# bkpcoding/distributed_ML_pytorch

Measured on AMD Instinct MI355X. Metric: samples/sec (whole node) ResNet-18 ASGD at 1/2/4/8 MI355X; time-to-target-loss, higher is better.
Workload: dtype bf16; 1 GPU; model=resnet18 (CIFAR stem), global_batch=512, per_gpu_batch=512, image=3x32x32, parallelism=asgd-local-ps x1, n_push=10, n_pull=10, staleness=1, push_combine=sum, hip_graph=True, master_dtype=fp32, wire_dtype=fp32

## Files before the change

### distributed_ml_pytorch_amd/csrc/bind/norm_pool.cpp

```cpp
#include "util.h"

namespace dmp::bind {
namespace {

int64_t channels_of(const Tensor& x) { return x.size(1); }

using OptTensors = std::initializer_list<const optional<Tensor>*>;

void check_bn_stats(const Tensor& stats, int64_t C) {
  TORCH_CHECK(stats.scalar_type() == at::kFloat && stats.numel() == 4 * C,
              "bn: stats must be fp32 [4, C]");
}

struct BnFwd {
  int64_t C, M;
  at::TensorOptions fopt;
  Tensor y, stats, mask;
  std::vector<Tensor> result() const { return {y, stats, mask}; }
};

BnFwd bn_fwd_front(const Tensor& x, const optional<Tensor>& res, OptTensors affine, bool relu,
                   bool want_mask) {
  check_nhwc_bf16(x, "x");
  BnFwd f;
  f.C = channels_of(x);
  f.M = x.numel() / f.C;
  TORCH_CHECK(f.C % 8 == 0 && f.C <= 2048, "bn: C must be a multiple of 8 and <= 2048, got ", f.C);
  if (has(res)) {
    check_nhwc_bf16(*res, "res");
    same_shape(*res, x, "res");
  }
  check_vecs(affine, at::kFloat, f.C, "bn affine / running tensors");
  f.fopt = x.options().dtype(at::kFloat);
  f.y = at::empty_like(x);
  f.stats = at::empty({4, f.C}, f.fopt);
  if (want_mask && relu) f.mask = at::empty({f.M, f.C / 8}, x.options().dtype(at::kByte));
  return f;
}

std::vector<Tensor> bn_fwd(Tensor x, optional<Tensor> res, optional<Tensor> gamma,
                           optional<Tensor> beta, optional<Tensor> running_mean,
                           optional<Tensor> running_var, double momentum, double eps,
                           bool training, bool relu, optional<Tensor> slots, bool want_mask) {
  TORCH_CHECK(training || (has(running_mean) && has(running_var)),
// ... 72 lines not shown
  b.mask = relu_mask_ptr(mask, relu, b.M, b.C);
  b.fopt = x.options().dtype(at::kFloat);
  b.dx = at::empty_like(x);
  if (want_dres) b.dres = at::empty_like(x);
  return b;
}

std::vector<Tensor> bn_bwd(Tensor x, Tensor dy, optional<Tensor> y, optional<Tensor> gamma,
                           Tensor stats, optional<Tensor> dgamma, optional<Tensor> dbeta,
                           bool relu, bool want_dres, optional<Tensor> slots,
                           optional<Tensor> mask, bool batch_stats) {
  auto b = bn_bwd_front(x, dy, y, gamma, stats, dgamma, dbeta, relu, want_dres, mask);
  auto part = bn_slots(slots, b.C, b.fopt);
  auto coef = at::empty({3, b.C}, b.fopt);
  dmp::launch_bn_bwd(bf16(x), bf16(dy), b.y, ptr_or_null<float>(gamma), stats.data_ptr<float>(),
                     ptr_or_null<float>(dgamma), ptr_or_null<float>(dbeta), coef.data_ptr<float>(),
                     part.data_ptr<float>(), bf16(b.dx), bf16_or_null(b.dres), b.M, (int)b.C, relu,
                     cur_stream(), b.mask, batch_stats);
  return b.result();
}

std::vector<Tensor> bn_bwd_fold(Tensor x, Tensor dy, optional<Tensor> y, optional<Tensor> gamma,
                                Tensor stats, optional<Tensor> dgamma, optional<Tensor> dbeta,
                                bool relu, bool want_dres, Tensor slots, optional<Tensor> mask,
                                optional<Tensor> zero_buf) {
  auto b = bn_bwd_front(x, dy, y, gamma, stats, dgamma, dbeta, relu, want_dres, mask);
  auto part = bn_slots(slots, b.C, b.fopt);
  float* zb = other_slots(zero_buf, b.C, b.fopt, part);
  dmp::launch_bn_bwd_fold(bf16(x), bf16(dy), b.y, ptr_or_null<float>(gamma),
                          stats.data_ptr<float>(), ptr_or_null<float>(dgamma),
                          ptr_or_null<float>(dbeta), part.data_ptr<float>(), zb, bf16(b.dx),
                          bf16_or_null(b.dres), b.M, (int)b.C, relu, cur_stream(), b.mask);
  return b.result();
}

std::vector<Tensor> bn_relu_maxpool_fwd(Tensor x, Tensor part, bool have_partials,
                                        optional<Tensor> gamma, optional<Tensor> beta,
                                        optional<Tensor> running_mean,
                                        optional<Tensor> running_var, double momentum, double eps,
                                        optional<Tensor> zero_buf, int64_t K, int64_t S,
                                        int64_t P) {
  check_nhwc_bf16(x, "x");
  TORCH_CHECK(x.dim() == 4, "bn_relu_maxpool expects 4-D input");
  TORCH_CHECK(dmp::guard::bf16_bytes_ok(x.size(0), x.size(2), x.size(3), x.size(1)),
              "bn_relu_maxpool: x over 2 GiB (32-bit offsets)");
  const int N = (int)x.size(0), C = (int)x.size(1), H = (int)x.size(2), W = (int)x.size(3);
  TORCH_CHECK(dmp::bn_maxpool_supported(C, (int)K, (int)S, (int)P),
              "bn_relu_maxpool: needs C % 64 == 0, C <= 2048 and a 3x3/s2/p1 window");
  auto fopt = x.options().dtype(at::kFloat);
  part = bn_slots(part, C, fopt);
  float* zb = other_slots(zero_buf, C, fopt, part);
  check_vecs({&gamma, &beta, &running_mean, &running_var}, at::kFloat, C,
             "bn affine / running tensors");
  const int Ho = dmp::maxpool_out(H, (int)K, (int)S, (int)P);
  const int Wo = dmp::maxpool_out(W, (int)K, (int)S, (int)P);
  TORCH_CHECK(Ho > 0 && Wo > 0, "bn_relu_maxpool: window larger than input");
  auto y = at::empty({N, C, Ho, Wo}, x.options().memory_format(kCL));
  auto idx = at::empty({N, C, Ho, Wo}, x.options().dtype(at::kByte).memory_format(kCL));
  auto xm = at::empty({N, C, Ho, Wo}, x.options().memory_format(kCL));
  auto stats = at::empty({4, C}, fopt);
  dmp::launch_bn_relu_maxpool_fold(
      bf16(x), bf16(y), idx.data_ptr<uint8_t>(), bf16(xm), ptr_or_null<float>(gamma),
      ptr_or_null<float>(beta), ptr_or_null<float>(running_mean), ptr_or_null<float>(running_var),
      stats.data_ptr<float>(), part.data_ptr<float>(), zb, N, H, W, C, (float)momentum, (float)eps,
      have_partials, cur_stream());
  return {y, idx, stats, xm};
// ... 174 lines not shown
  if (!aligned(dy)) dy = dy.clone(mf);
  TORCH_CHECK(dy.sizes() == y.sizes() && dy.scalar_type() == at::kBFloat16, "relu_bwd: dy shape");
  Tensor dst = has(out) ? *out : at::empty_like(dy);
  TORCH_CHECK(dst.sizes() == y.sizes() && dst.is_contiguous(mf) &&
                  dst.scalar_type() == at::kBFloat16,
              "relu_bwd: out layout");
  Tensor dx = aligned(dst) ? dst : at::empty_like(dy);
  dmp::launch_relu_bwd(bf16(dy), bf16(y), bf16(dx), y.numel(), cur_stream());
  if (!dx.is_same(dst)) dst.copy_(dx);
  return dst;
}

}

void bind_norm_pool(pybind11::module_& m) {
  m.def("bn_fold_weights", &bn_fold_weights,
        "inference-time BatchNorm fold: (bf16 w * s, fp32 shift, bf16 shift)", py::arg("w"),
        py::arg("gamma"), py::arg("beta"), py::arg("rmean"), py::arg("rvar"),
        py::arg("cbias") = py::none(), py::arg("eps") = 1e-5);
  m.def("bn_fwd_from_partials", &bn_fwd_from_partials, "BN forward from conv-epilogue partials",
        py::arg("x"), py::arg("part"), py::arg("G"), py::arg("res"), py::arg("gamma"),
        py::arg("beta"), py::arg("running_mean"), py::arg("running_var"), py::arg("momentum"),
        py::arg("eps"), py::arg("relu"), py::arg("want_mask") = false);
  m.def("bn_fwd_fold", &bn_fwd_fold, "BN forward, finalize folded into the apply",
        py::arg("x"), py::arg("part"), py::arg("have_partials"), py::arg("res") = py::none(),
        py::arg("gamma") = py::none(), py::arg("beta") = py::none(),
        py::arg("running_mean") = py::none(), py::arg("running_var") = py::none(),
        py::arg("momentum") = 0.1, py::arg("eps") = 1e-5, py::arg("relu") = false,
        py::arg("want_mask") = false, py::arg("zero_buf") = py::none());
  m.def("bn_bwd_fold", &bn_bwd_fold, "BN backward, finalize folded into the apply",
        py::arg("x"), py::arg("dy"), py::arg("y"), py::arg("gamma"), py::arg("stats"),
        py::arg("dgamma"), py::arg("dbeta"), py::arg("relu"), py::arg("want_dres"),
        py::arg("slots"), py::arg("mask") = py::none(), py::arg("zero_buf") = py::none());
  m.def("bn_maxpool_supported",
        [](int64_t C, int64_t K, int64_t S, int64_t P) {
          return dmp::bn_maxpool_supported((int)C, (int)K, (int)S, (int)P);
        },
        "fused BN + ReLU + max pool applies to (C, K, S, P)");
  m.def("bn_relu_maxpool_fwd", &bn_relu_maxpool_fwd,
        "BN + ReLU + max pool forward, finalize folded in -> (y, idx, stats, x at the taps)",
        py::arg("x"),
        py::arg("part"), py::arg("have_partials"), py::arg("gamma"), py::arg("beta"),
        py::arg("running_mean"), py::arg("running_var"), py::arg("momentum"), py::arg("eps"),
        py::arg("zero_buf"), py::arg("K"), py::arg("S"), py::arg("P"));
  m.def("maxpool_bn_bwd", &maxpool_bn_bwd, "backward of bn_relu_maxpool_fwd -> dx", py::arg("x"),
        py::arg("dp"), py::arg("idx"), py::arg("xm"), py::arg("gamma"), py::arg("stats"), py::arg("dgamma"),
        py::arg("dbeta"), py::arg("slots"), py::arg("zero_buf"), py::arg("K"), py::arg("S"),
        py::arg("P"));
  m.def("bn_fwd", &bn_fwd, "NHWC batchnorm(+residual)(+relu) forward", py::arg("x"),
        py::arg("res"), py::arg("gamma"), py::arg("beta"), py::arg("running_mean"),
        py::arg("running_var"), py::arg("momentum"), py::arg("eps"), py::arg("training"),
        py::arg("relu"), py::arg("slots") = py::none(), py::arg("want_mask") = false);
  m.def("bn_bwd", &bn_bwd, "NHWC batchnorm(+residual)(+relu) backward", py::arg("x"),
        py::arg("dy"), py::arg("y"), py::arg("gamma"), py::arg("stats"), py::arg("dgamma"),
        py::arg("dbeta"), py::arg("relu"), py::arg("want_dres"), py::arg("slots") = py::none(),
        py::arg("mask") = py::none(), py::arg("batch_stats") = true);
  m.def("relu_bwd", &relu_bwd, "ReLU backward from the saved output", py::arg("dy"), py::arg("y"),
        py::arg("out") = py::none());
  m.def("gap_fwd", &gap_fwd, "NHWC global average pool forward");
  m.def("gap_linear_fwd", &gap_linear_fwd, "fused NHWC global average pool + Linear forward",
        py::arg("x"), py::arg("w"), py::arg("bias") = py::none());
  m.def("gap_linear_bwd", &gap_linear_bwd, "fused GAP + Linear backward (dx, dW +=, db +=)",
        py::arg("dy"), py::arg("f"), py::arg("w"), py::arg("gw"), py::arg("gb") = py::none(),
        py::arg("H"), py::arg("W"));
  m.def("gap_linear_supported",
        [](int64_t C, int64_t N) { return dmp::gap_linear_supported((int)C, (int)N); },
// ... 12 lines not shown
```

### distributed_ml_pytorch_amd/csrc/bn.hip

```cpp
#include "common.h"

#include <algorithm>
#include <cstdlib>

namespace dmp {

__device__ __forceinline__ void load8(const u16* p, float v[8]) {
  const bf16x8 r = *reinterpret_cast<const bf16x8*>(p);
#pragma unroll
  for (int k = 0; k < 8; ++k) v[k] = bf2f(r.v[k]);
}

__device__ __forceinline__ void store8(u16* p, const float v[8]) {
  bf16x8 r;
#pragma unroll
  for (int k = 0; k < 8; ++k) r.v[k] = f2bf(v[k]);
  *reinterpret_cast<bf16x8*>(p) = r;
}

__device__ __forceinline__ bf16x8 bn_ldv(const u16* p) { return *reinterpret_cast<const bf16x8*>(p); }
__device__ __forceinline__ void bn_stv(u16* p, const bf16x8& r) { *reinterpret_cast<bf16x8*>(p) = r; }

__device__ __forceinline__ void relu_mask_bits(unsigned bits, float g[8]) {
#pragma unroll
  for (int k = 0; k < 8; ++k) g[k] = (bits >> k) & 1u ? g[k] : 0.f;
}
__device__ __forceinline__ void relu_mask_from_x(const float xv[8], const float* __restrict__ stats,
                                                 int C, int c0, float g[8]) {
#pragma unroll
  for (int k = 0; k < 8; ++k) {
    const float y = fmaxf(bn_pre(xv[k], stats[2 * C + c0 + k], stats[3 * C + c0 + k]), 0.f);
    g[k] = bf2f(f2bf(y)) > 0.f ? g[k] : 0.f;
  }
// ... 656 lines not shown
#define DMP_BN_PART(R)                                                                          \
  hipLaunchKernelGGL((bn_partial_kernel<1, R>), dim3(G), dim3(256), lds, s, x, dy, y, mask, stats, \
                     part, M, C)
  if (mode == 0) DMP_BN_PART(0);
  else if (mode == 1) DMP_BN_PART(1);
  else if (mode == 2) DMP_BN_PART(2);
  else DMP_BN_PART(3);
#undef DMP_BN_PART
  const int cs = fold_cs(C);
  const dim3 grid = fold_grid(M, C, cs);
#define DMP_FOLD_B(CS, R, D)                                                                   \
  hipLaunchKernelGGL((bn_bwd_apply_fold_kernel<CS, R, D>), grid, dim3(256), 0, s, x, dy, y, mask, \
                     part, zero_buf, gamma, stats, dgamma, dbeta, dx, dres, M, C)
#define DMP_FOLD_BV(CS)                                                \
  if (dres) {                                                          \
    if (mode == 0) DMP_FOLD_B(CS, 0, true);                            \
    else if (mode == 1) DMP_FOLD_B(CS, 1, true);                       \
    else if (mode == 2) DMP_FOLD_B(CS, 2, true);                       \
    else DMP_FOLD_B(CS, 3, true);                                      \
  } else {                                                             \
    if (mode == 0) DMP_FOLD_B(CS, 0, false);                           \
    else if (mode == 1) DMP_FOLD_B(CS, 1, false);                      \
    else if (mode == 2) DMP_FOLD_B(CS, 2, false);                      \
    else DMP_FOLD_B(CS, 3, false);                                     \
  }
  if (cs == 64) { DMP_FOLD_BV(64) }
  else if (cs == 32) { DMP_FOLD_BV(32) }
  else if (cs == 16) { DMP_FOLD_BV(16) }
  else { DMP_FOLD_BV(8) }
#undef DMP_FOLD_BV
#undef DMP_FOLD_B
}

typedef unsigned int bnu32x4 __attribute__((ext_vector_type(4)));
typedef unsigned int bnu32x2 __attribute__((ext_vector_type(2)));
constexpr unsigned kBnOOB = 0x80000000u;
__device__ __forceinline__ __amdgpu_buffer_rsrc_t bn_rsrc(const void* p, long long bytes) {
  return __builtin_amdgcn_make_buffer_rsrc(const_cast<void*>(p), 0, (int)bytes, 0x00020000);
}
__device__ __forceinline__ bf16x8 bn_ld16(__amdgpu_buffer_rsrc_t rs, unsigned off) {
  return __builtin_bit_cast(bf16x8, __builtin_amdgcn_raw_buffer_load_b128(rs, off, 0, 0));
}
__device__ __forceinline__ uint2 bn_ld8(__amdgpu_buffer_rsrc_t rs, unsigned off) {
  const bnu32x2 v = __builtin_amdgcn_raw_buffer_load_b64(rs, off, 0, 0);
  return make_uint2(v.x, v.y);
}

template <int K, int S, int P>
struct PoolGather {
  static constexpr int KS = (K + S - 1) / S;
  bf16x8 gv[KS][KS];
  uint2 iv[KS][KS];
  bf16x8 xr;
  int h, w, hlo, hhi, wlo, whi;

  __device__ __forceinline__ void load(__amdgpu_buffer_rsrc_t rsx, __amdgpu_buffer_rsrc_t rsdp,
                                       __amdgpu_buffer_rsrc_t rsidx, int row, bool live, int H,
                                       int W, int C, int Ho, int Wo, int cofs) {
    w = row % W;
    const int r = row / W;
    h = r % H;
    const int n = r / H;
    hlo = max(0, (h + P - K + S) / S);
    hhi = live ? min(Ho - 1, (h + P) / S) : -1;
    wlo = max(0, (w + P - K + S) / S);
    whi = min(Wo - 1, (w + P) / S);
// ... 325 lines not shown
```

### distributed_ml_pytorch_amd/csrc/launchers.h

```cpp
#pragma once
#include <hip/hip_runtime_api.h>

#include "bn_slots.h"
#include <stdint.h>

namespace dmp {

void launch_asgd_fused_step(const float* g, float* p, float* acc, float* mom, uint16_t* w16,
                            long long n, float lr, float wd, float momentum, float dampening,
                            bool nesterov, hipStream_t s);
int optim_hyper_words();
void launch_optim_hyper(float* hyper, const float* g, float* partial, long long n, hipStream_t s);
void launch_asgd_fused_step_dev(const float* g, float* p, float* acc, float* mom, uint16_t* w16,
                                long long n, const float* hyper, float wd, float momentum,
                                float dampening, bool nesterov, hipStream_t s,
                                float* ema = nullptr);
void launch_adamw_fused_step(const float* g, float* p, float* acc, float* m, float* v,
                             uint16_t* w16, const uint8_t* decay, long long n, const float* hyper,
                             float wd, float eps, hipStream_t s, float* ema = nullptr);
void launch_arena_swap(float* p, float* e, uint16_t* w16, long long n, hipStream_t s);
void launch_ema_buffers(const long long* table, int rows, float* flat, long long flat_numel,
                        const float* hyper, int mode, hipStream_t s);
struct Wire {
  enum Kind { kF32, kBF16, kMX8 } kind;
// ... 47 lines not shown
                                 int ignore_index, hipStream_t s);

bool batch_assemble_staged(const void* data, int H, int W, int C);
void launch_batch_assemble(const uint8_t* data, const long long* labels, const uint16_t* lut,
                           const int* index, int count, int N, int H, int W, int C,
                           uint16_t* out_x, long long* out_y, signed char* draws, int pad,
                           bool flip, unsigned long long seed, uint32_t epoch, int path,
                           hipStream_t s);
void launch_batch_assemble_mix(const uint8_t* data, const long long* labels, const uint16_t* lut,
                               const int* index, int count, int N, int H, int W, int C,
                               uint16_t* out_x, long long* out_y, long long* out_y2,
                               float* out_lam, signed char* draws, int pad, bool flip,
                               unsigned long long seed, uint32_t epoch, float pix_lam,
                               float label_lam, int y0, int y1, int x0, int x1, int path,
                               hipStream_t s);

int bn_num_partials(long long M, int C);
void launch_bn_fold_weights(const float* w, const float* gamma, const float* beta,
                            const float* rmean, const float* rvar, const float* cbias,
                            uint16_t* w16, float* b32, uint16_t* b16, long long n, int CO,
                            float eps, hipStream_t s);
void launch_bn_fwd(const uint16_t* x, const uint16_t* res, uint16_t* y, const float* gamma,
                   const float* beta, float* running_mean, float* running_var, float* stats,
                   float* part, long long M, int C, float momentum, float eps, bool training,
                   bool relu, hipStream_t s, uint8_t* mask = nullptr);
void launch_bn_fwd_fold(const uint16_t* x, const uint16_t* res, uint16_t* y, const float* gamma,
                        const float* beta, float* running_mean, float* running_var, float* stats,
                        float* part, float* zero_buf, long long M, int C, float momentum,
                        float eps, bool relu, bool have_partials, hipStream_t s, uint8_t* mask);
void launch_bn_bwd_fold(const uint16_t* x, const uint16_t* dy, const uint16_t* y,
                        const float* gamma, const float* stats, float* dgamma, float* dbeta,
                        float* part, float* zero_buf, uint16_t* dx, uint16_t* dres, long long M,
                        int C, bool relu, hipStream_t s, const uint8_t* mask);
bool bn_maxpool_supported(int C, int K, int S, int P);
void launch_bn_relu_maxpool_fold(const uint16_t* x, uint16_t* y, uint8_t* idx, uint16_t* xm,
                                 const float* gamma,
                                 const float* beta, float* running_mean, float* running_var,
                                 float* stats, float* part, float* zero_buf, int N, int H, int W,
                                 int C, float momentum, float eps, bool have_partials,
                                 hipStream_t s);
void launch_maxpool_bn_bwd_fold(const uint16_t* x, const uint16_t* dp, const uint8_t* idx,
                                const uint16_t* xm, const float* gamma, const float* stats, float* dgamma,
                                float* dbeta, float* part, float* zero_buf, uint16_t* dx, int N,
                                int H, int W, int C, hipStream_t s);
void launch_bn_bwd(const uint16_t* x, const uint16_t* dy, const uint16_t* y, const float* gamma,
                   const float* stats, float* dgamma, float* dbeta, float* coef, float* part,
                   uint16_t* dx, uint16_t* dres, long long M, int C, bool relu, hipStream_t s,
                   const uint8_t* mask = nullptr, bool batch_stats = true);

void launch_gap_fwd(const uint16_t* x, uint16_t* y, int N, int HW, int C, hipStream_t s);
void launch_gap_bwd(const uint16_t* dy, uint16_t* dx, int N, int HW, int C, hipStream_t s);
bool gap_linear_supported(int C, int N);
void launch_gap_linear_fwd(const uint16_t* x, const uint16_t* w, const uint16_t* bias, uint16_t* y,
                           uint16_t* f, int B, int HW, int C, int N, hipStream_t s);
void launch_gap_linear_bwd(const uint16_t* dy, const uint16_t* f, const uint16_t* w, uint16_t* dx,
                           float* gw, float* gb, int B, int HW, int C, int N, hipStream_t s);
int maxpool_out(int H, int K, int S, int P);
void launch_maxpool_fwd(const uint16_t* x, uint16_t* y, uint8_t* idx, int N, int H, int W, int C,
                        int K, int S, int P, hipStream_t s, bool nchw_out = false,
                        bool relu_in = false);
void launch_maxpool_bwd(const uint16_t* dy, const uint8_t* idx, uint16_t* dx, int N, int H,
                        int W, int C, int K, int S, int P, hipStream_t s, bool nchw_dy = false);


bool layernorm_supported(int D);
int layernorm_num_slots();
// ... 154 lines not shown
```

### distributed_ml_pytorch_amd/models/resnet.py

```python
from __future__ import annotations

import os

import torch
import torch.nn as nn

from ..ops import layers as L
from ..ops.eval_fold import conv_bn, fold_enabled
from ..ops.functional import bn_relu_maxpool, bn_relu_maxpool_ok, mark_residual_only
from ..ops.linear import gap_linear, gap_linear_ok


_SC_SUB = os.environ.get("DMP_SC_SUB", "1") != "0"


def _sc_sub(shortcut) -> bool:
    return (shortcut is not None and _SC_SUB and shortcut[0].kernel_size == (1, 1)
            and shortcut[0].stride == (2, 2) and shortcut[0].padding == (0, 0))


class BasicBlock(nn.Module):
    expansion = 1

    def __init__(self, cin: int, planes: int, stride: int = 1):
        super().__init__()
        self.conv1 = L.Conv2d(cin, planes, 3, stride=stride, padding=1, bias=False)
        self.bn1 = L.BatchNorm2d(planes, relu=True)
        self.conv2 = L.Conv2d(planes, planes, 3, stride=1, padding=1, bias=False)
        self.bn2 = L.BatchNorm2d(planes, relu=True)
        self.shortcut = None
        if stride != 1 or cin != planes:
            self.shortcut = nn.Sequential(
                L.Conv2d(cin, planes, 1, stride=stride, bias=False), L.BatchNorm2d(planes))

    def _forward_folded(self, x):
        h = conv_bn(x, self.conv1, self.bn1)
        if h is None:
            return None
        sc = x if self.shortcut is None else conv_bn(x, self.shortcut[0], self.shortcut[1])
        if sc is None:
            return None
        return conv_bn(h, self.conv2, self.bn2, residual=sc)

    def forward(self, x):
        if fold_enabled(x, self):
            y = self._forward_folded(x)
            if y is not None:
                return y
        sub = self.conv1.stride == (2, 2) and _sc_sub(self.shortcut)
        h, xa = self.conv1(x, alias="sub" if sub else True)
        h = self.bn1(h)
        if self.shortcut is None:
            sc = xa
        elif sub and xa.shape[-1] != x.shape[-1]:
            sc = self.shortcut[1](self.shortcut[0](xa, stride=1))
        else:
            sc = self.shortcut(xa)
        return self.bn2(self.conv2(h), residual=sc if sc is x else mark_residual_only(sc))


class Bottleneck(nn.Module):
    expansion = 4

    def __init__(self, cin: int, planes: int, stride: int = 1):
        super().__init__()
        out = planes * self.expansion
        self.conv1 = L.Conv2d(cin, planes, 1, bias=False)
        self.bn1 = L.BatchNorm2d(planes, relu=True)
        self.conv2 = L.Conv2d(planes, planes, 3, stride=stride, padding=1, bias=False)
        self.bn2 = L.BatchNorm2d(planes, relu=True)
        self.conv3 = L.Conv2d(planes, out, 1, bias=False)
        self.bn3 = L.BatchNorm2d(out, relu=True)
        self.shortcut = None
        if stride != 1 or cin != out:
            self.shortcut = nn.Sequential(
                L.Conv2d(cin, out, 1, stride=stride, bias=False), L.BatchNorm2d(out))

    def _forward_folded(self, x):
        h = conv_bn(x, self.conv1, self.bn1)
        h = conv_bn(h, self.conv2, self.bn2) if h is not None else None
        if h is None:
            return None
        sc = x if self.shortcut is None else conv_bn(x, self.shortcut[0], self.shortcut[1])
        if sc is None:
            return None
        return conv_bn(h, self.conv3, self.bn3, residual=sc)

    def forward(self, x):
        if fold_enabled(x, self):
            y = self._forward_folded(x)
            if y is not None:
                return y
        sub = _sc_sub(self.shortcut)
        h, xa = self.conv1(x, alias="sub" if sub else True)
        h = self.bn2(self.conv2(self.bn1(h)))
        if self.shortcut is None:
            sc = xa
        elif sub and xa.shape[-1] != x.shape[-1]:
            sc = self.shortcut[1](self.shortcut[0](xa, stride=1))
        else:
            sc = self.shortcut(xa)
        return self.bn3(self.conv3(h), residual=sc if sc is x else mark_residual_only(sc))


class ResNet(nn.Module):
    def __init__(self, block, layers, num_classes: int = 10, stem: str = "cifar",
                 zero_init_residual: bool = False):
        super().__init__()
        self.stem_kind = stem
        if stem == "cifar":
            self.conv1 = L.Conv2d(3, 64, 3, stride=1, padding=1, bias=False)
            self.pool = None
        elif stem == "imagenet":
            self.conv1 = L.Conv2d(3, 64, 7, stride=2, padding=3, bias=False)
            self.pool = L.MaxPool2d(3, stride=2, padding=1)
        else:
            raise ValueError(f"unknown stem {stem!r}")
        self.bn1 = L.BatchNorm2d(64, relu=True)
        cin = 64
        stages = []
        for i, (planes, n) in enumerate(zip((64, 128, 256, 512), layers)):
            blocks = []
            for j in range(n):
                stride = 2 if (i > 0 and j == 0) else 1
                blocks.append(block(cin, planes, stride))
                cin = planes * block.expansion
            stages.append(nn.Sequential(*blocks))
        self.layer1, self.layer2, self.layer3, self.layer4 = stages
        self.avgpool = L.GlobalAvgPool()
        self.linear = L.Linear(cin, num_classes)
        for m in self.modules():
            if isinstance(m, nn.Conv2d):
                nn.init.kaiming_normal_(m.weight, mode="fan_out", nonlinearity="relu")
            if isinstance(m, L.Conv2d):
                m.emit_bn_stats = True
# ... 40 lines not shown
```

### distributed_ml_pytorch_amd/ops/functional.py

```python
from __future__ import annotations

import os

import torch
import torch.nn.functional as F
from torch.autograd import Function

from ._ext import native
from ._grads import GradSink, notify
from ._policy import stock_gpu

CL = torch.channels_last


def mark_relu_masked(t):
    if t is not None:
        t._dmp_relu_masked_ver = t._version
    return t


def is_relu_masked(t) -> bool:
    return t is not None and getattr(t, "_dmp_relu_masked_ver", None) == t._version


# ... 288 lines not shown
        if ctx.fold:
            if x.dim() == 4:
                dy = dy.contiguous(memory_format=CL)
            else:
                dy = dy.contiguous()
            bs = _fresh_slots(ctx.bslots, x.shape[1], x.device)
            if in_mask is not None:
                DEFER_RES_STATS["native"] += 1
                dx, dres = native().bn_bwd_fold(x, dy, None, gamma, stats, dg, db, True, False,
                                                bs, in_mask, ctx.fpart)
            else:
                dx, dres = native().bn_bwd_fold(x, dy, y, gamma, stats, dg, db, ctx.relu,
                                                ctx.has_res and not ctx.defer_res, bs, mask,
                                                ctx.fpart)
                if ctx.defer_res:
                    dres = defer_tag(dy, mask)
                    DEFER_RES_STATS["deferred"] += 1
            mark_slots(bs, True)
            mark_slots(ctx.fpart, False)
            ctx.fpart = None
        else:
            if x.dim() == 4:
                dy = dy.contiguous(memory_format=CL)
            else:
                dy = dy.contiguous()
            if ctx.bslots is not None:
                clean_slots(ctx.bslots)
            dx, dres = native().bn_bwd(x, dy, y, gamma, stats, dg, db, ctx.relu, ctx.has_res,
                                       ctx.bslots, mask, ctx.training)
        return (dx, sg.done(), sb.done(), (dres if ctx.has_res else None), None, None, None, None,
                None, None, None, None, None)


def batch_norm_act(x, weight, bias, running_mean, running_var, training: bool, momentum: float,
                   eps: float, relu: bool = False, residual=None, slots=None):
    if x.is_cuda and x.dtype == torch.bfloat16 and x.shape[1] % 8 == 0 and x.shape[1] <= 2048:
        if not training and (running_mean is None or running_var is None):
            training = True
        part = getattr(x, "_dmp_bn_part", None) if training else None
        stem = getattr(x, "_dmp_stem", None) if (training and relu and residual is None
                                                   and part is not None) else None
        return _BNAct.apply(x, weight, bias, residual, running_mean, running_var, training,
                            momentum, eps, relu, part, slots, stem)
    if x.is_cuda and x.dtype == torch.bfloat16:
        raise RuntimeError(
            f"batch_norm_act: unsupported bf16 GPU input (C={x.shape[1]}); "
            "the native kernel needs C % 8 == 0 and C <= 2048")
    stock_gpu("batch_norm", x)
    w = weight.to(x.dtype) if weight is not None else None
    b = bias.to(x.dtype) if bias is not None else None
    y = F.batch_norm(x, running_mean, running_var, w, b, training, momentum, eps)
    if residual is not None:
        y = y + residual
    return F.relu(y) if relu else y


class _GAP(Function):
    @staticmethod
    def forward(ctx, x):
        x = x.contiguous(memory_format=CL)
        ctx.hw = (x.shape[2], x.shape[3])
        return native().gap_fwd(x)

    @staticmethod
    def backward(ctx, dy):
        return native().gap_bwd(dy.contiguous(), ctx.hw[0], ctx.hw[1])
# ... 519 lines not shown
```

Baseline: 143,300 samples/s.

## Fuse main-path and shortcut BatchNorms into one dual BN kernel in downsample blocks

Adds dual BatchNorm forward and backward kernels for residual blocks with a conv+BN shortcut. The forward computes relu(bn2(y2) + bn_s(ys)) in one pass, so the shortcut BN output is never materialised. The backward computes both layers' gradient partials and applies them in one shared pass over dy and the mask. This saves kernel launches and a round trip through memory for the shortcut activation. It only applies to the three downsample blocks in ResNet-18, and it adds extra atomics and registers in the fused kernels.

```diff
diff --git a/distributed_ml_pytorch_amd/csrc/bind/norm_pool.cpp b/distributed_ml_pytorch_amd/csrc/bind/norm_pool.cpp
--- a/distributed_ml_pytorch_amd/csrc/bind/norm_pool.cpp
+++ b/distributed_ml_pytorch_amd/csrc/bind/norm_pool.cpp
@@ -8,8 +8,9 @@
 using OptTensors = std::initializer_list<const optional<Tensor>*>;
 
 void check_bn_stats(const Tensor& stats, int64_t C) {
-  TORCH_CHECK(stats.scalar_type() == at::kFloat && stats.numel() == 4 * C,
-              "bn: stats must be fp32 [4, C]");
+  TORCH_CHECK(stats.is_cuda() && stats.scalar_type() == at::kFloat && stats.is_contiguous() &&
+                  stats.numel() == 4 * C,
+              "bn: stats must be a contiguous fp32 GPU tensor [4, C]");
 }
 
 struct BnFwd {
@@ -148,6 +149,75 @@
                           ptr_or_null<float>(dbeta), part.data_ptr<float>(), zb, bf16(b.dx),
                           bf16_or_null(b.dres), b.M, (int)b.C, relu, cur_stream(), b.mask);
   return b.result();
+}
+
+void check_dual_slots(const Tensor& part2, const Tensor& parts, const float* zb2,
+                      const float* zbs) {
+  const float* p2 = part2.data_ptr<float>();
+  const float* ps = parts.data_ptr<float>();
+  TORCH_CHECK(p2 != ps, "bn dual: the two layers share one slot buffer");
+  for (const float* zb : {zb2, zbs})
+    TORCH_CHECK(zb == nullptr || (zb != p2 && zb != ps),
+                "bn fold: zero_buf must not alias the slots being reduced");
+  TORCH_CHECK(zb2 == nullptr || zb2 != zbs, "bn dual: the two layers share one zero_buf");
+}
+
+std::vector<Tensor> bn_dual_fwd(Tensor y2, Tensor ys, Tensor part2, bool have_partials2,
+                                Tensor parts, bool have_partialss, optional<Tensor> gamma2,
+                                optional<Tensor> beta2, optional<Tensor> running_mean2,
+                                optional<Tensor> running_var2, double momentum2, double eps2,
+                                optional<Tensor> gammas, optional<Tensor> betas,
+                                optional<Tensor> running_means, optional<Tensor> running_vars,
+                                double momentums, double epss, optional<Tensor> zero_buf2,
+                                optional<Tensor> zero_bufs) {
+  auto f = bn_fwd_front(y2, ys, {&gamma2, &beta2, &running_mean2, &running_var2, &gammas, &betas,
+                                 &running_means, &running_vars}, true, true);
+  part2 = bn_slots(part2, f.C, f.fopt);
+  parts = bn_slots(parts, f.C, f.fopt);
+  float* zb2 = other_slots(zero_buf2, f.C, f.fopt, part2);
+  float* zbs = other_slots(zero_bufs, f.C, f.fopt, parts);
+  check_dual_slots(part2, parts, zb2, zbs);
+  auto statss = at::empty({4, f.C}, f.fopt);
+  const dmp::BnFoldFwd a{ptr_or_null<float>(gamma2), ptr_or_null<float>(beta2),
+                         ptr_or_null<float>(running_mean2), ptr_or_null<float>(running_var2),
+                         f.stats.data_ptr<float>(), part2.data_ptr<float>(), zb2,
+                         (float)momentum2, (float)eps2, have_partials2};
+  const dmp::BnFoldFwd b{ptr_or_null<float>(gammas), ptr_or_null<float>(betas),
+                         ptr_or_null<float>(running_means), ptr_or_null<float>(running_vars),
+                         statss.data_ptr<float>(), parts.data_ptr<float>(), zbs,
+                         (float)momentums, (float)epss, have_partialss};
+  dmp::launch_bn_dual_fwd_fold(bf16(y2), bf16(ys), a, b, bf16(f.y), f.mask.data_ptr<uint8_t>(),
+                               f.M, (int)f.C, cur_stream());
+  return {f.y, f.mask, f.stats, statss};
+}
+
+std::vector<Tensor> bn_dual_bwd(Tensor y2, Tensor ys, Tensor dy, Tensor mask,
+                                optional<Tensor> gamma2, Tensor stats2, optional<Tensor> dgamma2,
+                                optional<Tensor> dbeta2, Tensor slots2, optional<Tensor> zero_buf2,
+                                optional<Tensor> gammas, Tensor statss, optional<Tensor> dgammas,
+                                optional<Tensor> dbetas, Tensor slotss,
+                                optional<Tensor> zero_bufs) {
+  check_nhwc_bf16(ys, "ys");
+  same_shape(ys, y2, "ys");
+  auto b2 = bn_bwd_front(y2, dy, c10::nullopt, gamma2, stats2, dgamma2, dbeta2, true, false, mask);
+  TORCH_CHECK(b2.mask != nullptr, "bn dual: the backward needs the forward's ReLU mask");
+  check_bn_stats(statss, b2.C);
+  check_vecs({&gammas, &dgammas, &dbetas}, at::kFloat, b2.C, "bn gamma / dgamma / dbeta");
+  auto part2 = bn_slots(slots2, b2.C, b2.fopt);
+  auto parts = bn_slots(slotss, b2.C, b2.fopt);
+  float* zb2 = other_slots(zero_buf2, b2.C, b2.fopt, part2);
+  float* zbs = other_slots(zero_bufs, b2.C, b2.fopt, parts);
+  check_dual_slots(part2, parts, zb2, zbs);
+  auto dys = at::empty_like(ys);
+  const dmp::BnFoldBwd a{ptr_or_null<float>(gamma2), stats2.data_ptr<float>(),
+                         ptr_or_null<float>(dgamma2), ptr_or_null<float>(dbeta2),
+                         part2.data_ptr<float>(), zb2, bf16(b2.dx)};
+  const dmp::BnFoldBwd b{ptr_or_null<float>(gammas), statss.data_ptr<float>(),
+                         ptr_or_null<float>(dgammas), ptr_or_null<float>(dbetas),
+                         parts.data_ptr<float>(), zbs, bf16(dys)};
+  dmp::launch_bn_dual_bwd_fold(bf16(y2), bf16(ys), bf16(dy), b2.mask, a, b, b2.M, (int)b2.C,
+                               cur_stream());
+  return {b2.dx, dys};
 }
 
 std::vector<Tensor> bn_relu_maxpool_fwd(Tensor x, Tensor part, bool have_partials,
@@ -388,6 +458,18 @@
         py::arg("x"), py::arg("dy"), py::arg("y"), py::arg("gamma"), py::arg("stats"),
         py::arg("dgamma"), py::arg("dbeta"), py::arg("relu"), py::arg("want_dres"),
         py::arg("slots"), py::arg("mask") = py::none(), py::arg("zero_buf") = py::none());
+  m.def("bn_dual_fwd", &bn_dual_fwd,
+        "relu(bn2(y2) + bn_s(ys)) in one pass -> (out, mask, stats2, statss)", py::arg("y2"),
+        py::arg("ys"), py::arg("part2"), py::arg("have_partials2"), py::arg("parts"),
+        py::arg("have_partialss"), py::arg("gamma2"), py::arg("beta2"), py::arg("running_mean2"),
+        py::arg("running_var2"), py::arg("momentum2"), py::arg("eps2"), py::arg("gammas"),
+        py::arg("betas"), py::arg("running_means"), py::arg("running_vars"), py::arg("momentums"),
+        py::arg("epss"), py::arg("zero_buf2") = py::none(), py::arg("zero_bufs") = py::none());
+  m.def("bn_dual_bwd", &bn_dual_bwd, "backward of bn_dual_fwd -> (dy2, dys)", py::arg("y2"),
+        py::arg("ys"), py::arg("dy"), py::arg("mask"), py::arg("gamma2"), py::arg("stats2"),
+        py::arg("dgamma2"), py::arg("dbeta2"), py::arg("slots2"), py::arg("zero_buf2"),
+        py::arg("gammas"), py::arg("statss"), py::arg("dgammas"), py::arg("dbetas"),
+        py::arg("slotss"), py::arg("zero_bufs"));
   m.def("bn_maxpool_supported",
         [](int64_t C, int64_t K, int64_t S, int64_t P) {
           return dmp::bn_maxpool_supported((int)C, (int)K, (int)S, (int)P);
diff --git a/distributed_ml_pytorch_amd/csrc/bn.hip b/distributed_ml_pytorch_amd/csrc/bn.hip
--- a/distributed_ml_pytorch_amd/csrc/bn.hip
+++ b/distributed_ml_pytorch_amd/csrc/bn.hip
@@ -1,4 +1,5 @@
 #include "common.h"
+#include "launchers.h"
 
 #include <algorithm>
 #include <cstdlib>
@@ -721,6 +722,246 @@
 #undef DMP_FOLD_B
 }
 
+template <int CS>
+__global__ void __launch_bounds__(256) __attribute__((amdgpu_waves_per_eu(5)))
+bn_dual_apply_fold_kernel(
+    const u16* __restrict__ y2, const u16* __restrict__ ys, const BnFoldFwd a, const BnFoldFwd b,
+    u16* __restrict__ out, uint8_t* __restrict__ mask, long long M, int C) {
+  __shared__ float lS2[CS], lQ2[CS], lSs[CS], lQs[CS];
+  const int t = threadIdx.x;
+  const int cs0 = blockIdx.y * CS;
+  fold_fwd_coefs<CS>(b.part, b.zero_buf, b.gamma, b.beta, b.running_mean, b.running_var,
+                     b.momentum, b.eps, b.stats, M, C, cs0, lSs, lQs);
+  fold_fwd_coefs<CS>(a.part, a.zero_buf, a.gamma, a.beta, a.running_mean, a.running_var,
+                     a.momentum, a.eps, a.stats, M, C, cs0, lS2, lQ2);
+  constexpr int TPR = CS / 8, RPI = 256 / TPR;
+  const int cg = t % TPR, r0 = t / TPR;
+  float sc2[8], sh2[8], scs[8], shs[8];
+#pragma unroll
+  for (int k = 0; k < 8; ++k) {
+    sc2[k] = lS2[cg * 8 + k]; sh2[k] = lQ2[cg * 8 + k];
+    scs[k] = lSs[cg * 8 + k]; shs[k] = lQs[cg * 8 + k];
+  }
+  const long long rows_per_blk = (M + gridDim.x - 1) / gridDim.x;
+  const long long start = (long long)blockIdx.x * rows_per_blk;
+  const long long end = min(M, start + rows_per_blk);
+  auto one = [&](const bf16x8& xr, const bf16x8& sr, long long off) {
+    bf16x8 r;
+    unsigned bits = 0;
+#pragma unroll
+    for (int k = 0; k < 8; ++k) {
+      const float sv = bf2f(f2bf(bn_pre(bf2f(sr.v[k]), scs[k], shs[k])));
+      float o = bn_pre(bf2f(xr.v[k]), sc2[k], sh2[k]);
+      o += sv;
+      o = fmaxf(o, 0.f);
+      r.v[k] = f2bf(o);
+      bits |= (r.v[k] != 0 ? 1u : 0u) << k;
+    }
+    bn_stv(out + off, r);
+    mask[off >> 3] = (uint8_t)bits;
+  };
+  constexpr int U = 4;
+  long long row = start + r0;
+  const int cofs = cs0 + cg * 8;
+  for (; row + (U - 1) * RPI < end; row += U * RPI) {
+    bf16x8 xr[U], sr[U];
+#pragma unroll
+    for (int u = 0; u < U; ++u) {
+      const long long off = (row + u * RPI) * C + cofs;
+      xr[u] = bn_ldv(y2 + off);
+      sr[u] = bn_ldv(ys + off);
+    }
+#pragma unroll
+    for (int u = 0; u < U; ++u) one(xr[u], sr[u], (row + u * RPI) * C + cofs);
+  }
+  for (; row < end; row += RPI) {
+    const long long off = row * C + cofs;
+    one(bn_ldv(y2 + off), bn_ldv(ys + off), off);
+  }
+}
+
+__global__ void __launch_bounds__(256) bn_dual_partial_kernel(
+    const u16* __restrict__ x2, const u16* __restrict__ xs, const u16* __restrict__ dy,
+    const uint8_t* __restrict__ mask, const float* __restrict__ stats2,
+    const float* __restrict__ statss, float* __restrict__ part2, float* __restrict__ parts,
+    long long M, int C) {
+  extern __shared__ __attribute__((aligned(16))) float smem[];
+  const int tpr = C >> 3;
+  const int rpi = 256 / tpr;
+  const int t = threadIdx.x;
+  const int cg = t % tpr, r0 = t / tpr;
+  const long long rows_per_blk = (M + gridDim.x - 1) / gridDim.x;
+  const long long start = (long long)blockIdx.x * rows_per_blk;
+  const long long end = min(M, start + rows_per_blk);
+  float s[8], q2[8], qs[8], mean2[8], inv2[8], means[8], invs[8];
+#pragma unroll
+  for (int k = 0; k < 8; ++k) {
+    s[k] = 0.f; q2[k] = 0.f; qs[k] = 0.f;
+    mean2[k] = stats2[cg * 8 + k]; inv2[k] = stats2[C + cg * 8 + k];
+    means[k] = statss[cg * 8 + k]; invs[k] = statss[C + cg * 8 + k];
+  }
+  auto accum = [&](const bf16x8& ar, const bf16x8& br, const bf16x8& dr, unsigned mb) {
+    float g[8];
+#pragma unroll
+    for (int k = 0; k < 8; ++k) g[k] = bf2f(dr.v[k]);
+    relu_mask_bits(mb, g);
+#pragma unroll
+    for (int k = 0; k < 8; ++k) {
+      const float av = bf2f(ar.v[k]), bv = bf2f(br.v[k]);
+      s[k] += g[k];
+      q2[k] += g[k] * (av - mean2[k]) * inv2[k];
+      qs[k] += g[k] * (bv - means[k]) * invs[k];
+    }
+  };
+  constexpr int U = 4;
+  if (r0 < rpi) {
+    long long row = start + r0;
+    for (; row + (U - 1) * rpi < end; row += U * rpi) {
+      bf16x8 ar[U], br[U], dr[U];
+      unsigned mb[U];
+#pragma unroll
+      for (int u = 0; u < U; ++u) {
+        const long long off = (row + u * rpi) * C + cg * 8;
+        ar[u] = bn_ldv(x2 + off);
+        br[u] = bn_ldv(xs + off);
+        dr[u] = bn_ldv(dy + off);
+        mb[u] = mask[off >> 3];
+      }
+#pragma unroll
+      for (int u = 0; u < U; ++u) accum(ar[u], br[u], dr[u], mb[u]);
+    }
+    for (; row < end; row += rpi) {
+      const long long off = row * C + cg * 8;
+      accum(bn_ldv(x2 + off), bn_ldv(xs + off), bn_ldv(dy + off), mask[off >> 3]);
+    }
+  }
+  float* ls = smem;
+  float* l2 = smem + rpi * C;
+  float* lb = smem + 2 * rpi * C;
+  if (r0 < rpi) {
+#pragma unroll
+    for (int k = 0; k < 8; ++k) {
+      ls[r0 * C + cg * 8 + k] = s[k];
+      l2[r0 * C + cg * 8 + k] = q2[k];
+      lb[r0 * C + cg * 8 + k] = qs[k];
+    }
+  }
+  __syncthreads();
+  for (int c = t; c < C; c += 256) {
+    float a = 0.f, b = 0.f, d = 0.f;
+    for (int r = 0; r < rpi; ++r) { a += ls[r * C + c]; b += l2[r * C + c]; d += lb[r * C + c]; }
+    const int slot = blockIdx.x % kBnSlots;
+    atomicAdd(part2 + (long long)slot * C + c, a);
+    atomicAdd(part2 + (long long)(kBnSlots + slot) * C + c, b);
+    atomicAdd(parts + (long long)slot * C + c, a);
+    atomicAdd(parts + (long long)(kBnSlots + slot) * C + c, d);
+  }
+}
+
+template <int CS>
+__global__ void __launch_bounds__(256) bn_dual_bwd_apply_fold_kernel(
+    const u16* __restrict__ x2, const u16* __restrict__ xs, const u16* __restrict__ dy,
+    const uint8_t* __restrict__ mask, const BnFoldBwd a, const BnFoldBwd b, long long M, int C) {
+  __shared__ float lS2[CS], lQ2[CS], lC2[CS], lSs[CS], lQs[CS], lCs[CS];
+  const int t = threadIdx.x;
+  const int cs0 = blockIdx.y * CS;
+  fold_bwd_coefs<CS>(a.part, a.zero_buf, a.gamma, a.stats, a.dgamma, a.dbeta, M, C, cs0, lS2, lQ2,
+                     lC2);
+  fold_bwd_coefs<CS>(b.part, b.zero_buf, b.gamma, b.stats, b.dgamma, b.dbeta, M, C, cs0, lSs, lQs,
+                     lCs);
+  constexpr int TPR = CS / 8, RPI = 256 / TPR;
+  const int cg = t % TPR, r0 = t / TPR;
+  const int cofs = cs0 + cg * 8;
+  float ka2[8], kb2[8], kc2[8], kas[8], kbs[8], kcs[8];
+#pragma unroll
+  for (int k = 0; k < 8; ++k) {
+    ka2[k] = lS2[cg * 8 + k]; kb2[k] = lQ2[cg * 8 + k]; kc2[k] = lC2[cg * 8 + k];
+    kas[k] = lSs[cg * 8 + k]; kbs[k] = lQs[cg * 8 + k]; kcs[k] = lCs[cg * 8 + k];
+  }
+  u16* __restrict__ dx2 = a.dx;
+  u16* __restrict__ dxs = b.dx;
+  const long long rows_per_blk = (M + gridDim.x - 1) / gridDim.x;
+  const long long start = (long long)blockIdx.x * rows_per_blk;
+  const long long end = min(M, start + rows_per_blk);
+  auto one = [&](const bf16x8& ar, const bf16x8& br, const bf16x8& dr, unsigned mb,
+                 long long off) {
+    float g[8], o2[8], os[8];
+#pragma unroll
+    for (int k = 0; k < 8; ++k) g[k] = bf2f(dr.v[k]);
+    relu_mask_bits(mb, g);
+#pragma unroll
+    for (int k = 0; k < 8; ++k) {
+      o2[k] = ka2[k] * g[k] + kc2[k] * bf2f(ar.v[k]) + kb2[k];
+      os[k] = kas[k] * g[k] + kcs[k] * bf2f(br.v[k]) + kbs[k];
+    }
+    store8(dx2 + off, o2);
+    store8(dxs + off, os);
+  };
+  constexpr int U = 4;
+  long long row = start + r0;
+  for (; row + (U - 1) * RPI < end; row += U * RPI) {
+    bf16x8 ar[U], br[U], dr[U];
+    unsigned mb[U];
+#pragma unroll
+    for (int u = 0; u < U; ++u) {
+      const long long off = (row + u * RPI) * C + cofs;
+      ar[u] = bn_ldv(x2 + off);
+      br[u] = bn_ldv(xs + off);
+      dr[u] = bn_ldv(dy + off);
+      mb[u] = mask[off >> 3];
+    }
+#pragma unroll
+    for (int u = 0; u < U; ++u) one(ar[u], br[u], dr[u], mb[u], (row + u * RPI) * C + cofs);
+  }
+  for (; row < end; row += RPI) {
+    const long long off = row * C + cofs;
+    one(bn_ldv(x2 + off), bn_ldv(xs + off), bn_ldv(dy + off), mask[off >> 3], off);
+  }
+}
+
+void launch_bn_dual_fwd_fold(const u16* y2, const u16* ys, const BnFoldFwd& main,
+                             const BnFoldFwd& sc, u16* out, uint8_t* mask, long long M, int C,
+                             hipStream_t s) {
+  const int rpi = 256 / (C / 8);
+  const size_t lds = (size_t)rpi * C * 2 * sizeof(float);
+  if (!sc.have_partials)
+    hipLaunchKernelGGL((bn_partial_kernel<0, 0>), dim3(bn_num_partials(M, C)), dim3(256), lds, s,
+                       ys, nullptr, nullptr, nullptr, nullptr, sc.part, M, C);
+  if (!main.have_partials)
+    hipLaunchKernelGGL((bn_partial_kernel<0, 0>), dim3(bn_num_partials(M, C)), dim3(256), lds, s,
+                       y2, nullptr, nullptr, nullptr, nullptr, main.part, M, C);
+  const int cs = fold_cs(C);
+  const dim3 grid = fold_grid(M, C, cs);
+#define DMP_DUAL_F(CS)                                                                       \
+  hipLaunchKernelGGL((bn_dual_apply_fold_kernel<CS>), grid, dim3(256), 0, s, y2, ys, main, sc, \
+                     out, mask, M, C)
+  if (cs == 64) DMP_DUAL_F(64);
+  else if (cs == 32) DMP_DUAL_F(32);
+  else if (cs == 16) DMP_DUAL_F(16);
+  else DMP_DUAL_F(8);
+#undef DMP_DUAL_F
+}
+
+void launch_bn_dual_bwd_fold(const u16* y2, const u16* ys, const u16* dy, const uint8_t* mask,
+                             const BnFoldBwd& main, const BnFoldBwd& sc, long long M, int C,
+                             hipStream_t s) {
+  const int G = bn_bwd_partials(M, C);
+  const int rpi = 256 / (C / 8);
+  const size_t lds = (size_t)rpi * C * 3 * sizeof(float);
+  hipLaunchKernelGGL(bn_dual_partial_kernel, dim3(G), dim3(256), lds, s, y2, ys, dy, mask,
+                     main.stats, sc.stats, main.part, sc.part, M, C);
+  const int cs = fold_cs(C);
+  const dim3 grid = fold_grid(M, C, cs);
+#define DMP_DUAL_B(CS)                                                                         \
+  hipLaunchKernelGGL((bn_dual_bwd_apply_fold_kernel<CS>), grid, dim3(256), 0, s, y2, ys, dy, mask, \
+                     main, sc, M, C)
+  if (cs == 64) DMP_DUAL_B(64);
+  else if (cs == 32) DMP_DUAL_B(32);
+  else if (cs == 16) DMP_DUAL_B(16);
+  else DMP_DUAL_B(8);
+#undef DMP_DUAL_B
+}
+
 typedef unsigned int bnu32x4 __attribute__((ext_vector_type(4)));
 typedef unsigned int bnu32x2 __attribute__((ext_vector_type(2)));
 constexpr unsigned kBnOOB = 0x80000000u;
diff --git a/distributed_ml_pytorch_amd/csrc/launchers.h b/distributed_ml_pytorch_amd/csrc/launchers.h
--- a/distributed_ml_pytorch_amd/csrc/launchers.h
+++ b/distributed_ml_pytorch_amd/csrc/launchers.h
@@ -103,6 +103,32 @@
                         const float* gamma, const float* stats, float* dgamma, float* dbeta,
                         float* part, float* zero_buf, uint16_t* dx, uint16_t* dres, long long M,
                         int C, bool relu, hipStream_t s, const uint8_t* mask);
+struct BnFoldFwd {
+  const float* gamma;
+  const float* beta;
+  float* running_mean;
+  float* running_var;
+  float* stats;
+  float* part;
+  float* zero_buf;
+  float momentum, eps;
+  bool have_partials;
+};
+struct BnFoldBwd {
+  const float* gamma;
+  const float* stats;
+  float* dgamma;
+  float* dbeta;
+  float* part;
+  float* zero_buf;
+  uint16_t* dx;
+};
+void launch_bn_dual_fwd_fold(const uint16_t* y2, const uint16_t* ys, const BnFoldFwd& main,
+                             const BnFoldFwd& sc, uint16_t* out, uint8_t* mask, long long M,
+                             int C, hipStream_t s);
+void launch_bn_dual_bwd_fold(const uint16_t* y2, const uint16_t* ys, const uint16_t* dy,
+                             const uint8_t* mask, const BnFoldBwd& main, const BnFoldBwd& sc,
+                             long long M, int C, hipStream_t s);
 bool bn_maxpool_supported(int C, int K, int S, int P);
 void launch_bn_relu_maxpool_fold(const uint16_t* x, uint16_t* y, uint8_t* idx, uint16_t* xm,
                                  const float* gamma,
diff --git a/distributed_ml_pytorch_amd/models/resnet.py b/distributed_ml_pytorch_amd/models/resnet.py
--- a/distributed_ml_pytorch_amd/models/resnet.py
+++ b/distributed_ml_pytorch_amd/models/resnet.py
@@ -7,7 +7,8 @@
 
 from ..ops import layers as L
 from ..ops.eval_fold import conv_bn, fold_enabled
-from ..ops.functional import bn_relu_maxpool, bn_relu_maxpool_ok, mark_residual_only
+from ..ops.functional import (batch_norm_dual, bn_dual_ok, bn_relu_maxpool, bn_relu_maxpool_ok,
+                              mark_residual_only)
 from ..ops.linear import gap_linear, gap_linear_ok
 
 
@@ -17,6 +18,26 @@
 def _sc_sub(shortcut) -> bool:
     return (shortcut is not None and _SC_SUB and shortcut[0].kernel_size == (1, 1)
             and shortcut[0].stride == (2, 2) and shortcut[0].padding == (0, 0))
+
+
+def _conv_bn_pair(shortcut) -> bool:
+    return (isinstance(shortcut, nn.Sequential) and len(shortcut) == 2
+            and isinstance(shortcut[0], L.Conv2d) and isinstance(shortcut[1], L.BatchNorm2d))
+
+
+def _block_out(x, xa, sub, shortcut, last_conv, bn, h):
+    if shortcut is None:
+        sc = xa
+    elif _conv_bn_pair(shortcut):
+        conv, sbn = shortcut[0], shortcut[1]
+        ys = conv(xa, stride=1) if sub and xa.shape[-1] != x.shape[-1] else conv(xa)
+        y = last_conv(h)
+        if bn_dual_ok(y, ys, bn, sbn):
+            return batch_norm_dual(y, ys, bn, sbn)
+        return bn(y, residual=mark_residual_only(sbn(ys)))
+    else:
+        sc = shortcut(xa)
+    return bn(last_conv(h), residual=sc if sc is x else mark_residual_only(sc))
 
 
 class BasicBlock(nn.Module):
@@ -49,14 +70,7 @@
                 return y
         sub = self.conv1.stride == (2, 2) and _sc_sub(self.shortcut)
         h, xa = self.conv1(x, alias="sub" if sub else True)
-        h = self.bn1(h)
-        if self.shortcut is None:
-            sc = xa
-        elif sub and xa.shape[-1] != x.shape[-1]:
-            sc = self.shortcut[1](self.shortcut[0](xa, stride=1))
-        else:
-            sc = self.shortcut(xa)
-        return self.bn2(self.conv2(h), residual=sc if sc is x else mark_residual_only(sc))
+        return _block_out(x, xa, sub, self.shortcut, self.conv2, self.bn2, self.bn1(h))
 
 
 class Bottleneck(nn.Module):
@@ -94,13 +108,7 @@
         sub = _sc_sub(self.shortcut)
         h, xa = self.conv1(x, alias="sub" if sub else True)
         h = self.bn2(self.conv2(self.bn1(h)))
-        if self.shortcut is None:
-            sc = xa
-        elif sub and xa.shape[-1] != x.shape[-1]:
-            sc = self.shortcut[1](self.shortcut[0](xa, stride=1))
-        else:
-            sc = self.shortcut(xa)
-        return self.bn3(self.conv3(h), residual=sc if sc is x else mark_residual_only(sc))
+        return _block_out(x, xa, sub, self.shortcut, self.conv3, self.bn3, h)
 
 
 class ResNet(nn.Module):
diff --git a/distributed_ml_pytorch_amd/ops/functional.py b/distributed_ml_pytorch_amd/ops/functional.py
--- a/distributed_ml_pytorch_amd/ops/functional.py
+++ b/distributed_ml_pytorch_amd/ops/functional.py
@@ -344,6 +344,72 @@
                 None, None, None, None, None)
 
 
+_BN_DUAL = os.environ.get("DMP_BN_DUAL", "1") != "0"
+
+
+class _BNDual(Function):
+
+    @staticmethod
+    def forward(ctx, y2, ys, gamma2, beta2, gammas, betas, lay2, lays):
+        C = y2.shape[1]
+        srcs, bsl = [], []
+        for _, _, _, _, part, slots in (lay2, lays):
+            srcs.append(part if part is not None else _fresh_slots(
+                slots[0] if slots is not None else None, C, y2.device))
+            bsl.append(slots[1] if slots is not None else None)
+        out, mask, stats2, statss = native().bn_dual_fwd(
+            y2, ys, srcs[0], lay2[4] is not None, srcs[1], lays[4] is not None,
+            gamma2, beta2, lay2[0], lay2[1], float(lay2[2]), float(lay2[3]),
+            gammas, betas, lays[0], lays[1], float(lays[2]), float(lays[3]), bsl[0], bsl[1])
+        for src, b in zip(srcs, bsl):
+            mark_slots(src, True)
+            if b is not None:
+                mark_slots(b, False)
+        ctx.fparts, ctx.bslots = srcs, bsl
+        ctx.params = (gamma2, beta2, gammas, betas)
+        out._dmp_bn_out = True
+        ctx.save_for_backward(y2, ys, stats2, statss, mask)
+        return out
+
+    @staticmethod
+    def backward(ctx, dy):
+        y2, ys, stats2, statss, mask = ctx.saved_tensors
+        gamma2, beta2, gammas, betas = ctx.params
+        dy = resolve_deferred(dy).contiguous(memory_format=CL)
+        sinks = [GradSink(p, ctx.needs_input_grad[2 + i], dtype=None)
+                 for i, p in enumerate(ctx.params)]
+        bs = [_fresh_slots(b, y2.shape[1], y2.device) for b in ctx.bslots]
+        dy2, dys = native().bn_dual_bwd(
+            y2, ys, dy, mask, gamma2, stats2, sinks[0].buf, sinks[1].buf, bs[0], ctx.fparts[0],
+            gammas, statss, sinks[2].buf, sinks[3].buf, bs[1], ctx.fparts[1])
+        DEFER_RES_STATS["deferred"] += 1
+        DEFER_RES_STATS["native"] += 1
+        for b, src in zip(bs, ctx.fparts):
+            mark_slots(b, True)
+            mark_slots(src, False)
+        ctx.fparts = None
+        return (dy2, dys, *[s.done() for s in sinks], None, None)
+
+
+def bn_dual_ok(y2, ys, bn2, bns) -> bool:
+    return bool(_BN_DUAL and _BN_FOLD and _BN_DEFER_RES and _BN_BITMASK
+                and bn2.training and bns.training and bn2.relu and not bns.relu
+                and y2.is_cuda and y2.dtype == torch.bfloat16 and ys.dtype == torch.bfloat16
+                and y2.dim() == 4 and y2.shape == ys.shape
+                and y2.shape[1] % 8 == 0 and y2.shape[1] <= 2048
+                and y2.is_contiguous(memory_format=CL) and ys.is_contiguous(memory_format=CL))
+
+
+def batch_norm_dual(y2, ys, bn2, bns):
+    def layer(bn, x):
+        track = bn.track_running_stats
+        return (bn.running_mean if track else None, bn.running_var if track else None,
+                0.1 if bn.momentum is None else bn.momentum, bn.eps,
+                getattr(x, "_dmp_bn_part", None), bn._slots(x))
+    return _BNDual.apply(y2, ys, bn2.weight, bn2.bias, bns.weight, bns.bias, layer(bn2, y2),
+                         layer(bns, ys))
+
+
 def batch_norm_act(x, weight, bias, running_mean, running_var, training: bool, momentum: float,
                    eps: float, relu: bool = False, residual=None, slots=None):
     if x.is_cuda and x.dtype == torch.bfloat16 and x.shape[1] % 8 == 0 and x.shape[1] <= 2048:
```

Measured after the change: 144,700 samples/s (median of 6 runs). Within noise of the previous version (+1.0%).
